# faustomorales/keras-ocr

Measured on AMD Instinct MI355X. Metric: images/sec end-to-end Pipeline.recognize() @768x768, higher is better.
Workload: dtype f32 (fp32 operands as 2 fp16 pieces [F(4,3) / head layers] or 3 bf16 pieces [1x1, dilated], 3 / 6 MFMA products, fp32 accumulate; fp32-class error vs fp64: tests/test_conv_gpu.py)

## Files before the change

### keras_ocr_amd/csrc/api.cpp

```cpp
#include "abi.h"
#include "taps.h"
#include <cmath>
#include <algorithm>
#include <mutex>
#include <set>

int arena_reserve(kocr_ctx* ctx, Arena& a, size_t bytes) {
  ctx->last_pl.valid = false;
  if (bytes <= a.cap) return KOCR_OK;
  if (a.base) {
    KOCR_HIP(ctx, hipStreamSynchronize(ctx->stream));
    KOCR_HIP(ctx, hipFree(a.base));
    a.base = nullptr;
    a.cap = 0;
  }
  const size_t want = bytes + (bytes >> 3) + 4096;
  void* p = nullptr;
  hipError_t e = hipMalloc(&p, want);
  if (e != hipSuccess) {
    ctx->set_err("workspace hipMalloc(" + std::to_string(want) + " B) failed: " + hipGetErrorString(e));
    return KOCR_ENOMEM;
  }
  a.base = (char*)p;
  a.cap = want;
// ... 88 lines not shown
  pending.push_back(pd);
  ProfRow& r = prof[name];
  r.launches += 1;
  r.flops += flops;
  r.bytes += bytes;
}

void kocr_ctx::prof_end() { hipEventRecord(pending.back().b, stream); }

int kocr_ctx::prof_flush() {
  if (pending.empty()) return KOCR_OK;
  KOCR_HIP(this, hipStreamSynchronize(stream));
  for (Pending& pd : pending) {
    float ms = 0.f;
    hipEventElapsedTime(&ms, pd.a, pd.b);
    prof[pd.name].ms += ms;
    ev_pool.push_back(pd.a);
    ev_pool.push_back(pd.b);
  }
  pending.clear();
  return KOCR_OK;
}

int craft_micro_batch(int micro_batch, int N, int H, int W) {
  int mb = micro_batch > 0 ? micro_batch : 32;
  while (mb > 1 && craft_workspace_bytes(mb, H, W) > ((size_t)96 << 30)) mb = (mb + 1) / 2;
  return std::min(mb, N);
}

long prepare_box_warps(kocr_ctx* ctx, const char* fn, int N, const float* boxes, const int32_t* counts, const void* out, int th,
                       int tw, std::vector<WarpParam>& prm) {
  const std::string f(fn);
  long M = 0;
  for (int i = 0; i < N; ++i) {
    if (counts[i] < 0) KOCR_FAIL(ctx, KOCR_EINVAL, f + ": negative count");
    M += counts[i];
  }
  if (M == 0) return 0;
  if (!boxes || !out) KOCR_FAIL(ctx, KOCR_EINVAL, f + ": null buffer");
  prm.resize((size_t)M);
  long m = 0;
  for (int i = 0; i < N; ++i)
    for (int j = 0; j < counts[i]; ++j, ++m) {
      const int rc = warp_prepare(boxes + m * 8, th, tw, &prm[m], nullptr);
      if (rc == 1) KOCR_FAIL(ctx, KOCR_EZERODIV, f + ": box with zero width or height (ZeroDivisionError at tools.py:95)");
      if (rc != 0) KOCR_FAIL(ctx, KOCR_EINVAL, f + ": singular perspective transform");
      prm[m].img = i;
    }
  return M;
}

extern "C" {

int kocr_create(kocr_ctx** out, int hip_device) {
  if (!out) return KOCR_EINVAL;
  *out = nullptr;
  int count = 0;
  if (hipGetDeviceCount(&count) != hipSuccess || hip_device < 0 || hip_device >= count) return KOCR_EHIP;
  if (hipSetDevice(hip_device) != hipSuccess) return KOCR_EHIP;
  kocr_ctx* c = new kocr_ctx();
  if (const char* e = getenv("KOCR_SPLIT"))
    c->split_mode = (!strcmp(e, "f16") || !strcmp(e, "fp16") || !strcmp(e, "f16x2")) ? KOCR_SPLIT_F16X2
                    : (!strcmp(e, "f16x1") || !strcmp(e, "fast"))                     ? KOCR_SPLIT_F16X1
                                                                                      : KOCR_SPLIT_BF16X3;
  {
    auto on = [](const char* name, bool dflt) {
      const char* e = getenv(name);
      return e ? atoi(e) != 0 : dflt;
    };
    c->sw.dense_splitk = on("KOCR_DENSE_SPLITK", true);
    c->sw.lstm16 = on("KOCR_LSTM16", true);
    c->sw.hs16 = on("KOCR_HS16", true);
    c->sw.k5 = on("KOCR_K5", true);
    c->sw.up2x = on("KOCR_UP2X", true);
    c->sw.w43h = on("KOCR_W43H", true);
    c->sw.w43 = on("KOCR_W43", true);
    c->sw.w43r = on("KOCR_W43R", true);
    c->sw.w43v = on("KOCR_W43V", true);
    c->sw.w43rag = on("KOCR_W43RAG", true);
    c->sw.w43dilh = on("KOCR_W43DILH", true);
    c->sw.cells = on("KOCR_CELLS", true);
    c->sw.wsplit = on("KOCR_WSPLIT", true);
    c->sw.dsplit = on("KOCR_DSPLIT", true);
    c->sw.hsplit = on("KOCR_HSPLIT", true);
    c->sw.first = on("KOCR_FIRST", true);
  }
  c->prof_layers = getenv("KOCR_PROF_LAYERS") != nullptr;
  if (const char* e = getenv("KOCR_LINFOLD")) c->opt_linfold = atoi(e) != 0;
  if (const char* e = getenv("KOCR_UPFOLD")) c->opt_upfold = atoi(e) != 0;
  c->device = hip_device;
  if (hipDeviceGetAttribute(&c->n_cu, hipDeviceAttributeMultiprocessorCount, hip_device) != hipSuccess ||
      hipStreamCreateWithFlags(&c->own_stream, hipStreamNonBlocking) != hipSuccess) {
    delete c;
    return KOCR_EHIP;
  }
  c->stream = c->own_stream;
  *out = c;
  return KOCR_OK;
}

void kocr_destroy(kocr_ctx* ctx) {
  if (!ctx) return;
  hipSetDevice(ctx->device);
  hipStreamSynchronize(ctx->stream);
  craft_free(ctx);
  crnn_free(ctx);
  for (void* p : ctx->owned) hipFree(p);
  for (Arena* a : {&ctx->ws, &ctx->pp, &ctx->pp2, &ctx->io, &ctx->pl, &ctx->bx})
    if (a->base) hipFree(a->base);
  for (auto& pd : ctx->pending) {
    hipEventDestroy(pd.a);
    hipEventDestroy(pd.b);
  }
  for (hipEvent_t e : ctx->ev_pool) hipEventDestroy(e);
  hipStreamDestroy(ctx->own_stream);
  delete ctx;
}

const char* kocr_last_error(const kocr_ctx* ctx) { return ctx ? ctx->err.c_str() : "null ctx"; }

int kocr_set_stream(kocr_ctx* ctx, void* hip_stream) {
  if (!ctx) return KOCR_EINVAL;
  KOCR_HIP(ctx, hipStreamSynchronize(ctx->stream));
  ctx->stream = hip_stream ? (hipStream_t)hip_stream : ctx->own_stream;
  return KOCR_OK;
}

int kocr_synchronize(kocr_ctx* ctx) {
  if (!ctx) return KOCR_EINVAL;
  KOCR_HIP(ctx, hipStreamSynchronize(ctx->stream));
  return KOCR_OK;
}

int kocr_device_alloc(kocr_ctx* ctx, void** out, uint64_t bytes) {
  if (!ctx || !out) return KOCR_EINVAL;
  KOCR_HIP(ctx, hipSetDevice(ctx->device));
  KOCR_HIP(ctx, hipMalloc(out, bytes ? bytes : 4));
  return KOCR_OK;
}

int kocr_device_free(kocr_ctx* ctx, void* p) {
  if (!ctx) return KOCR_EINVAL;
  KOCR_HIP(ctx, hipStreamSynchronize(ctx->stream));
  KOCR_HIP(ctx, hipFree(p));
  return KOCR_OK;
}

int kocr_memcpy_h2d(kocr_ctx* ctx, void* dst, const void* src, uint64_t bytes) {
  if (!ctx) return KOCR_EINVAL;
  KOCR_HIP(ctx, hipMemcpyAsync(dst, src, bytes, hipMemcpyHostToDevice, ctx->stream));
  KOCR_HIP(ctx, hipStreamSynchronize(ctx->stream));
  return KOCR_OK;
}

int kocr_memcpy_d2h(kocr_ctx* ctx, void* dst, const void* src, uint64_t bytes) {
  if (!ctx) return KOCR_EINVAL;
  KOCR_HIP(ctx, hipMemcpyAsync(dst, src, bytes, hipMemcpyDeviceToHost, ctx->stream));
  KOCR_HIP(ctx, hipStreamSynchronize(ctx->stream));
  return KOCR_OK;
}

int kocr_load_craft(kocr_ctx* ctx, int n, const char* const* names, const float* const* data,
                    const int64_t* shapes, const int* ranks) {
  if (!ctx || n <= 0 || !names || !data || !shapes || !ranks) return KOCR_EINVAL;
  KOCR_HIP(ctx, hipSetDevice(ctx->device));
  return craft_load(ctx, n, names, data, shapes, ranks);
// ... 617 lines not shown
```

### keras_ocr_amd/csrc/common.h

```cpp
#pragma once
#include <hip/hip_runtime.h>
#include <stdint.h>
#include <string>
#include <vector>
#include <map>
#include <atomic>
#include <cstdio>
#include <cstring>
#include "../../include/kocr.h"

#define KOCR_HIP(ctx, expr)                                                         \
  do {                                                                              \
    hipError_t _e = (expr);                                                         \
    if (_e != hipSuccess) {                                                         \
      (ctx)->set_err(std::string(#expr) + ": " + hipGetErrorString(_e) + " at " +   \
                     __FILE__ + ":" + std::to_string(__LINE__));                    \
      return KOCR_EHIP;                                                             \
    }                                                                               \
  } while (0)

#define KOCR_TRY(expr)            \
  do {                            \
    int _rc = (expr);             \
    if (_rc != KOCR_OK) return _rc; \
  } while (0)

#define KOCR_FAIL(ctx, code, msg) \
  do {                            \
    (ctx)->set_err(msg);          \
    return (code);                \
  } while (0)

struct Tensor {
  float* p = nullptr;
  int N = 0, H = 0, W = 0, C = 0;
  int cs = 0;
  int co = 0;
  unsigned* amax = nullptr;
  int Wv = 0;
  int wv() const { return Wv ? Wv : W; }
  int cellW = 0, cellWv = 0;
  int cells() const { return cellW ? W / cellW : 0; }
  size_t pixels() const { return (size_t)N * H * W; }
  Tensor slice(int off, int c) const {
    Tensor t = *this;
    t.co = co + off;
    t.C = c;
    return t;
  }
};

struct ConvLayer {
  std::string name;
  int Cin = 0, Cout = 0, KH = 1, KW = 1, dil = 1;
  int Kreal = 0, Kpad = 0, Cout_pad = 0, BN = 0;
  float* d_w = nullptr;
  float* d_pre_a = nullptr;
  float* d_pre_b = nullptr;
  float* d_post_a = nullptr;
  float* d_post_b = nullptr;
  int relu = 0;
  float* d_w_rgb4 = nullptr;
  unsigned short* d_ws = nullptr;
  int ws_cout_pad = 0;
  unsigned short* d_w4 = nullptr;
  int w4_cout_pad = 0;
  unsigned short* d_w4h = nullptr;
  float* d_pre_a_h = nullptr;
  unsigned short* d_ds = nullptr;
  int ds_cout_pad = 0;
  unsigned short* d_first = nullptr;
  float first_bound = 0.f;
  unsigned short* d_hs = nullptr;
  unsigned short* d_hs16 = nullptr;
  unsigned short* d_hsh = nullptr;
  std::vector<int> hs_wexp;
  unsigned short* d_k5 = nullptr;
  bool tap_inner = false;
  bool ready() const { return d_w != nullptr; }
};

struct ProfRow {
  int64_t launches = 0;
  double ms = 0, flops = 0, bytes = 0;
};

struct RangeRow {
  double launches = 0, elements = 0, nonzero = 0, below_m4 = 0, below_m14 = 0, sum_abs = 0, sum_abs_below_m4 = 0;
};

struct Arena {
  char* base = nullptr;
  size_t cap = 0, off = 0;
};

struct CraftNet;
struct CrnnNet;
struct Taps;

struct kocr_ctx {
  int device = 0;
  hipStream_t own_stream = nullptr;
  hipStream_t stream = nullptr;
  std::string err;
  void set_err(const std::string& s) { err = s; }

  int split_mode = KOCR_SPLIT_F16X2;
  bool opt_linfold = true, opt_upfold = true;
  int min_area_rect = KOCR_RECT_EXACT;
  struct Switches {
    bool dense_splitk = true;
    bool lstm16 = true;
    bool hs16 = true;
    bool k5 = true;
    bool up2x = true;
    bool w43h = true;
    bool w43 = true;
    bool w43r = true;
    bool w43v = true;
    bool w43rag = true;
    bool w43dilh = true;
    bool cells = true;
    bool wsplit = true;
    bool dsplit = true;
    bool hsplit = true;
    bool first = true;
  } sw;
  bool prof_layers = false;
  int n_cu = 0;

  unsigned* d_amax = nullptr;
  int amax_used = 0;
  static constexpr int AMAX_SLOTS = 1 << 16;
  int amax_begin();
  unsigned* amax_slots(int n);

  Arena ws, pp, pp2, io, pl;
  Arena bx;
  int ws_reserve(size_t bytes);
  void ws_reset() { ws.off = 0; }
  void* ws_alloc(size_t bytes);

  std::vector<void*> owned;
  int dev_alloc(void** out, size_t bytes);
  int upload(float** out, const std::vector<float>& host);
  void release(void* p);

  CraftNet* craft = nullptr;
  CrnnNet* crnn = nullptr;
  Taps* taps = nullptr;
  std::vector<std::string>* tap_rows = nullptr;

  struct LastPipeline {
    const float* d_boxes = nullptr;
    const int32_t* d_counts = nullptr;
    const int32_t* d_labels = nullptr;
    int N = 0, cap = 0, M = 0;
    bool valid = false;
  } last_pl;

  bool range_on = false;
  void* d_range = nullptr;
  std::map<std::string, RangeRow> range;

  bool prof_on = false;
  std::map<std::string, ProfRow> prof;
  struct Pending {
    std::string name;
    hipEvent_t a, b;
  };
  std::vector<Pending> pending;
  std::vector<hipEvent_t> ev_pool;
  hipEvent_t get_event();
  void prof_begin(const char* name, double flops, double bytes);
  void prof_end();
  int prof_flush();
};

int arena_reserve(kocr_ctx* ctx, Arena& a, size_t bytes);
inline void* arena_alloc(Arena& a, size_t bytes) {
  const size_t o = (a.off + 255) & ~(size_t)255;
  if (o + bytes > a.cap) return nullptr;
  a.off = o + bytes;
  return a.base + o;
}
inline void* kocr_ctx::ws_alloc(size_t bytes) { return arena_alloc(ws, bytes); }

struct ProfScope {
  kocr_ctx* c;
  ProfScope(kocr_ctx* ctx, const char* name, double flops, double bytes) : c(ctx) {
    if (c->tap_rows) c->tap_rows->push_back(name);
    if (c->prof_on) c->prof_begin(name, flops, bytes);
  }
  ~ProfScope() {
    if (c->prof_on) c->prof_end();
  }
};

inline std::string prof_name(const kocr_ctx* ctx, const ConvLayer& L, const std::string& row, const std::string& layer_row) {
  return ctx->prof_layers ? layer_row + ":" + L.name : row;
}

template <auto K, typename P>
int launch_persistent(kocr_ctx* ctx, const P& p, int total_tiles, int block, int lds, int attr_lds, int occ = 1,
                      int* grid_out = nullptr) {
  static std::atomic<bool> attr_done[64];
  const int dev = ctx->device & 63;
// ... 162 lines not shown
```

### keras_ocr_amd/csrc/conv_dsplit.hip

```cpp
#include "split_common.h"
#include "w43_common.h"
#include "probe_clock.h"
#include <cmath>
#include <algorithm>

struct DsParams {
  const float* in;
  const unsigned short* wgt;
  float* out;
  const float* pre_a;
  const float* pre_b;
  const float* post_a;
  const float* post_b;
  int H, W, Cin, in_cs, in_co;
  int Cout, Cout_pad, out_cs, out_co;
  int relu;
  int KH, KW, dil;
  int nsteps;
  int Mtotal;
  int total_tiles;
  const unsigned* amax_in;
  int w_exp;
  unsigned* amax_out;
  const float* up;
  int up_H, up_W;
  float up_sy, up_sx;
  unsigned dv_hw[2];
};


template <int WM, int WN, int HALF, int UP, int PAIR = 0>
__global__ __launch_bounds__(128 * WM * WN, WM * WN == 2 ? 2 : 1) void conv_ds_kernel(DsParams p) {
  constexpr int NP = HALF ? 2 : 3;
  constexpr int NCW = WM * WN;
  constexpr int NMT = 8 * WM;
  constexpr int TILE_PX = 256 * WM;
  constexpr int PXI = 16 * NCW;
  constexpr int IPT = TILE_PX / PXI;
  constexpr int KH_STRIDE = 256;
  constexpr int PLANE = NMT * 2 * KH_STRIDE;
  constexpr int BUF = NP * PLANE;
  extern __shared__ __attribute__((aligned(16))) unsigned short As[];
  const int tid = threadIdx.x, lane = tid & 63;
  const int wave = __builtin_amdgcn_readfirstlane(tid >> 6);
  const int l31 = lane & 31, l5 = lane >> 5;
  const int nblk_n = p.Cout_pad / (32 * WN);
  const int total = p.total_tiles;
  const int ns = p.nsteps;
  const int G = gridDim.x;
  const int pad_y = p.dil * (p.KH / 2), pad_x = p.dil * (p.KW / 2);

  if (wave >= NCW) {
    const int ptid = tid - 64 * NCW;
    const int quad = ptid & 3;
    constexpr unsigned OOB = 0x80000000u;
    const float in_scale = HALF ? kocr_pow2(kocr_scale_exp(p.amax_in, 13)) : 1.f;
    (void)in_scale;
    int ldst[IPT];
#pragma unroll
    for (int it = 0; it < IPT; ++it) {
      const int idx = (ptid >> 2) + it * PXI;
      ldst[it] = ((idx >> 5) * 2 + (quad >> 1)) * KH_STRIDE + ((((idx & 31) * 8) ^ ((quad >> 1) * 32)) + (quad & 1) * 4);
    }
    int L_ld = blockIdx.x, ld_ky = 0, ld_kx = 0, ld_cg = 0;
    unsigned goff[IPT];
    int gy[IPT], gx[IPT];
    bool gok[IPT];
    __amdgpu_buffer_rsrc_t rsrc;
    auto tile_geometry = [&]() __attribute__((always_inline)) {
      const int tile = kocr_xcd_remap(L_ld < total ? L_ld : 0, total);
      const long pm0 = (long)(tile / nblk_n) * TILE_PX;
      const float* bbase_v = p.in + (pm0 * p.in_cs + p.in_co) - (long)(pad_y * p.W + pad_x) * p.in_cs;
      const unsigned long long bb = (unsigned long long)bbase_v;
      const unsigned long long bbu = ((unsigned long long)(unsigned)__builtin_amdgcn_readfirstlane((int)(bb >> 32)) << 32) |
                                     (unsigned)__builtin_amdgcn_readfirstlane((int)bb);
      rsrc = __builtin_amdgcn_make_buffer_rsrc((void*)bbu, 0, 0x80000000, 0x00020000);
#pragma unroll
      for (int it = 0; it < IPT; ++it) {
        const int idx = (ptid >> 2) + it * PXI;
        const long g = pm0 + idx;
        gok[it] = g < p.Mtotal && L_ld < total;
        gx[it] = (int)(g % p.W);
        gy[it] = (int)((g / p.W) % p.H);
        goff[it] = (unsigned)((idx * p.in_cs + quad * 4) * 4);
      }
    };
    auto load_raw2 = [&](v4f (&ra)[IPT], v4f (&rb)[IPT]) __attribute__((always_inline)) {
      const int soff = ld_cg * 64;
#pragma unroll
      for (int it = 0; it < IPT; ++it) {
        const unsigned off = gok[it] ? goff[it] : OOB;
        ra[it] = __builtin_bit_cast(v4f, __builtin_amdgcn_raw_buffer_load_b128(rsrc, off, soff, 0));
        rb[it] = __builtin_bit_cast(v4f, __builtin_amdgcn_raw_buffer_load_b128(rsrc, off, soff + 64, 0));
      }
      ld_cg += 2;
      if (ld_cg == p.Cin / 16) {
        ld_cg = 0;
        L_ld += G;
        tile_geometry();
      }
    };
    auto load_raw = [&](v4f (&raw)[IPT]) __attribute__((always_inline)) {
      const int dy = ld_ky * p.dil - pad_y, dx = ld_kx * p.dil - pad_x;
      const int soff = (((dy + pad_y) * p.W + (dx + pad_x)) * p.in_cs + ld_cg * 16) * 4;
#pragma unroll
      for (int it = 0; it < IPT; ++it) {
        const bool ok = gok[it] && (unsigned)(gy[it] + dy) < (unsigned)p.H && (unsigned)(gx[it] + dx) < (unsigned)p.W;
        raw[it] = __builtin_bit_cast(v4f, __builtin_amdgcn_raw_buffer_load_b128(rsrc, ok ? goff[it] : OOB, soff, 0));
      }
      if (++ld_kx == p.KW) {
        ld_kx = 0;
        if (++ld_ky == p.KH) {
          ld_ky = 0;
          if (++ld_cg == p.Cin / 16) {
            ld_cg = 0;
            L_ld += G;
            tile_geometry();
          }
        }
      }
    };
    auto produce = [&](const v4f (&raw)[IPT], int buf) __attribute__((always_inline)) {
      unsigned short* base = As + buf * BUF;
#pragma unroll
      for (int it = 0; it < IPT; ++it) {
        unsigned short* dst = base + ldst[it];
        if constexpr (HALF) {
          u2v h, l;
          kocr_split4_h(raw[it] * in_scale, h, l);
          *reinterpret_cast<u2v*>(dst) = h;
          *reinterpret_cast<u2v*>(dst + PLANE) = l;
        } else {
          u2v h, m, l;
          kocr_split4(raw[it], h, m, l);
          *reinterpret_cast<u2v*>(dst) = h;
          *reinterpret_cast<u2v*>(dst + PLANE) = m;
          *reinterpret_cast<u2v*>(dst + 2 * PLANE) = l;
        }
      }
    };
    const int my_tiles = (total - (int)blockIdx.x + G - 1) / G;
    const int T = my_tiles * ns;
    tile_geometry();
    constexpr int D = PAIR ? 6 : 4;
    v4f raw[D][IPT];
    int k = 0;
    if constexpr (PAIR) {
      load_raw2(raw[0], raw[1]);
      load_raw2(raw[2], raw[3]);
      PROBE_T0();
      for (; k + D <= T; k += D) {
#pragma unroll
        for (int d = 0; d < D; d += 2) {
          load_raw2(raw[(d + 4) % D], raw[(d + 5) % D]);
          PROBE_T(6);
          produce(raw[d], 0);
          PROBE_T(4);
          __syncthreads();
          PROBE_T(5);
          produce(raw[d + 1], 1);
          PROBE_T(4);
          __syncthreads();
          PROBE_T(5);
        }
      }
      PROBE_TEND(tid == 64 * NCW, 4, 7);
#pragma unroll
      for (int d = 0; d < 4; ++d)
        if (k + d < T) {
          produce(raw[d], d & 1);
          __syncthreads();
        }
    } else {
#pragma unroll
    for (int d = 0; d < D - 1; ++d) load_raw(raw[d]);
    PROBE_T0();
    for (; k + D <= T; k += D) {
#pragma unroll
      for (int d = 0; d < D; ++d) {
        load_raw(raw[(d + D - 1) % D]);
        PROBE_T(6);
        produce(raw[d], d & 1);
        PROBE_T(4);
        __syncthreads();
        PROBE_T(5);
      }
    }
    PROBE_TEND(tid == 64 * NCW, 4, 7);
#pragma unroll
    for (int d = 0; d < D - 1; ++d)
      if (k + d < T) {
        produce(raw[d], d & 1);
        __syncthreads();
      }
    }
    __syncthreads();
    return;
  }

  const int wn = (WN == 4) ? wave : (wave % WN), wm = (WM == 1) ? 0 : (wave / WN);
  const int ntiles32 = p.Cout_pad >> 5;
  const size_t w_step = (size_t)ntiles32 * NP * 64 * 8;
  auto w_tile = [&](int nt) { return p.wgt + ((size_t)(nt * WN + wn) * NP * 64 + lane) * 8; };

  bf8 bw[NP], bwn[NP];
  f16v acc[4][2];
  const int a_lane = (wm * 8 * 2 + l5) * KH_STRIDE + ((l31 * 8) ^ (l5 * 32));
  auto load_a = [&](bf8 (&a)[2][NP], const unsigned short* bufp, int g) __attribute__((always_inline)) {
    const unsigned short* base = bufp + a_lane + g * 4 * KH_STRIDE;
#pragma unroll
    for (int m = 0; m < 2; ++m)
#pragma unroll
      for (int s = 0; s < NP; ++s) a[m][s] = *reinterpret_cast<const bf8*>(base + s * PLANE + m * 2 * KH_STRIDE);
  };
  auto mfma6 = [&](const bf8 (&a)[2][NP], int g) __attribute__((always_inline)) {
    if constexpr (HALF) {
      const hf8 b0 = __builtin_bit_cast(hf8, bw[0]), b1 = __builtin_bit_cast(hf8, bw[1]);
#pragma unroll
      for (int m = 0; m < 2; ++m)
        acc[g][m] = __builtin_amdgcn_mfma_f32_32x32x16_f16(__builtin_bit_cast(hf8, a[m][1]), b0, acc[g][m], 0, 0, 0);
// ... 3 lines not shown
#pragma unroll
      for (int m = 0; m < 2; ++m)
        acc[g][m] = __builtin_amdgcn_mfma_f32_32x32x16_f16(__builtin_bit_cast(hf8, a[m][0]), b0, acc[g][m], 0, 0, 0);
    } else {
      const bf8 b0 = bw[0], b1 = bw[1], b2 = bw[NP - 1];
#pragma unroll
      for (int m = 0; m < 2; ++m) acc[g][m] = __builtin_amdgcn_mfma_f32_32x32x16_bf16(a[m][NP - 1], b0, acc[g][m], 0, 0, 0);
#pragma unroll
      for (int m = 0; m < 2; ++m) acc[g][m] = __builtin_amdgcn_mfma_f32_32x32x16_bf16(a[m][0], b2, acc[g][m], 0, 0, 0);
#pragma unroll
      for (int m = 0; m < 2; ++m) acc[g][m] = __builtin_amdgcn_mfma_f32_32x32x16_bf16(a[m][1], b1, acc[g][m], 0, 0, 0);
#pragma unroll
      for (int m = 0; m < 2; ++m) acc[g][m] = __builtin_amdgcn_mfma_f32_32x32x16_bf16(a[m][1], b0, acc[g][m], 0, 0, 0);
#pragma unroll
      for (int m = 0; m < 2; ++m) acc[g][m] = __builtin_amdgcn_mfma_f32_32x32x16_bf16(a[m][0], b1, acc[g][m], 0, 0, 0);
#pragma unroll
      for (int m = 0; m < 2; ++m) acc[g][m] = __builtin_amdgcn_mfma_f32_32x32x16_bf16(a[m][0], b0, acc[g][m], 0, 0, 0);
    }
  };
  bf8 a0[2][NP], a1[2][NP];
  auto compute_step = [&](auto last_c, const unsigned short* bufp, const unsigned short* bufn,
                          const unsigned short* w_next) __attribute__((always_inline)) {
    constexpr bool LAST = decltype(last_c)::value;
#pragma unroll
    for (int s = 0; s < NP; ++s) bwn[s] = *reinterpret_cast<const bf8*>(w_next + (size_t)s * 64 * 8);
    load_a(a1, bufp, 1);
    __builtin_amdgcn_sched_barrier(0);
    mfma6(a0, 0);
    __builtin_amdgcn_sched_barrier(0);
    load_a(a0, bufp, 2);
    __builtin_amdgcn_sched_barrier(0);
    mfma6(a1, 1);
    __builtin_amdgcn_sched_barrier(0);
    load_a(a1, bufp, 3);
    __builtin_amdgcn_sched_barrier(0);
    mfma6(a0, 2);
    __builtin_amdgcn_sched_barrier(0);
    __syncthreads();
    if constexpr (!LAST) load_a(a0, bufn, 0);
    __builtin_amdgcn_sched_barrier(0);
    mfma6(a1, 3);
    __builtin_amdgcn_sched_barrier(0);
#pragma unroll
    for (int s = 0; s < NP; ++s) bw[s] = bwn[s];
  };

  int gs = 0;
  {
    const int tile0 = kocr_xcd_remap(blockIdx.x, total);
    const unsigned short* w0 = w_tile(tile0 % nblk_n);
#pragma unroll
    for (int s = 0; s < NP; ++s) bw[s] = *reinterpret_cast<const bf8*>(w0 + (size_t)s * 64 * 8);
  }
  __syncthreads();
  load_a(a0, As, 0);
  PROBE_T0();
  for (int L = blockIdx.x; L < total; L += G) {
    const int tile = kocr_xcd_remap(L, total);
    const int mt = tile / nblk_n, nt = tile - mt * nblk_n;
    const long pm0 = (long)mt * TILE_PX;
    const unsigned short* w_ptr = w_tile(nt);
    const unsigned short* w_after = (L + G < total) ? w_tile(kocr_xcd_remap(L + G, total) % nblk_n) : w_ptr;
#pragma unroll
    for (int g = 0; g < 4; ++g)
#pragma unroll
      for (int m = 0; m < 2; ++m)
#pragma unroll
        for (int r = 0; r < 16; ++r) acc[g][m][r] = 0.f;
    __builtin_amdgcn_s_waitcnt(0x0F70);
    if constexpr (UP != 0) {
      for (int s = 0; s < ns - 1; ++s, ++gs)
        compute_step(std::false_type{}, As + (gs & 1) * BUF, As + ((gs + 1) & 1) * BUF, w_ptr + (size_t)(s + 1) * w_step);
      compute_step(std::true_type{}, As + (gs & 1) * BUF, As + ((gs + 1) & 1) * BUF, w_after);
      ++gs;
    } else {
      for (int s = 0; s < ns; ++s, ++gs)
        compute_step(std::false_type{}, As + (gs & 1) * BUF, As + ((gs + 1) & 1) * BUF, s + 1 < ns ? w_ptr + (size_t)(s + 1) * w_step : w_after);
    }
    PROBE_T(0);

    {
      const int n = (nt * WN + wn) * 32 + l31;
      const int nc = n < p.Cout ? n : p.Cout - 1;
      const float unscale = HALF ? kocr_pow2(-(kocr_scale_exp(p.amax_in, 13) + p.w_exp)) : 1.f;
      const float pa = p.pre_a[nc] * unscale, pb = p.pre_b[nc];
      const bool has_post = p.post_a != nullptr;
      const float qa = has_post ? p.post_a[nc] : 1.f, qb = has_post ? p.post_b[nc] : 0.f;
      if constexpr (UP) {
        unsigned* tab = reinterpret_cast<unsigned*>(As + 2 * BUF) + wave * (256 * 8);
        const long wbase = pm0 + (long)wm * 256;
        const unsigned ucs4 = (unsigned)p.Cout * 4u;
        const int hw = p.H * p.W;
        const long wb = wbase < (long)p.Mtotal - 1 ? wbase : (long)p.Mtotal - 1;
        const int n0 = __builtin_amdgcn_readfirstlane((int)(wb / hw));
#pragma unroll
        for (int i = 0; i < 4; ++i) {
          const int q = lane + 64 * i;
          long gl = wbase + q;
          if (gl > (long)p.Mtotal - 1) gl = (long)p.Mtotal - 1;
          const int gi = (int)gl;
          const int ox = gi % p.W, t2 = gi / p.W;
          const int oy = t2 % p.H, ni = t2 / p.H;
          const float fy = ((float)oy + 0.5f) * p.up_sy - 0.5f;
          const float fx = ((float)ox + 0.5f) * p.up_sx - 0.5f;
          const float fly = floorf(fy), flx = floorf(fx);
          const int y0 = max((int)fly, 0), y1 = min((int)ceilf(fy), p.up_H - 1);
          const int x0 = max((int)flx, 0), x1 = min((int)ceilf(fx), p.up_W - 1);
          const unsigned r0 = (unsigned)(((ni - n0) * p.up_H + y0) * p.up_W), r1 = (unsigned)(((ni - n0) * p.up_H + y1) * p.up_W);
          uint4 o4;
          o4.x = (r0 + x0) * ucs4;
          o4.y = (r0 + x1) * ucs4;
          o4.z = (r1 + x0) * ucs4;
          o4.w = (r1 + x1) * ucs4;
          *reinterpret_cast<uint4*>(tab + q * 8) = o4;
          float2 wl;
          wl.x = fx - flx;
          wl.y = fy - fly;
          *reinterpret_cast<float2*>(tab + q * 8 + 4) = wl;
        }
        __builtin_amdgcn_fence(__ATOMIC_SEQ_CST, "wavefront");
        __builtin_amdgcn_wave_barrier();
        const unsigned long long ub = (unsigned long long)(p.up + (size_t)n0 * p.up_H * p.up_W * p.Cout);
        const unsigned long long ubu = ((unsigned long long)(unsigned)__builtin_amdgcn_readfirstlane((int)(ub >> 32)) << 32) |
                                       (unsigned)__builtin_amdgcn_readfirstlane((int)ub);
        const __amdgpu_buffer_rsrc_t ru = __builtin_amdgcn_make_buffer_rsrc((void*)ubu, 0, 0x7FFFFFFF, 0x00020000);
        const unsigned ch = (unsigned)nc * 4u;
        if constexpr (UP == 2) {
          float tb[2][4][8];
          unsigned tab_lane = 4 * l5 * 8;
          asm volatile("" : "+v"(tab_lane));
          const unsigned* tab_l = tab + tab_lane;
          auto up_issue = [&](int gm, float (&v)[4][8]) __attribute__((always_inline)) {
#pragma unroll
            for (int rr = 0; rr < 4; ++rr) {
              const unsigned* e = tab_l + (gm * 32 + 8 * rr) * 8;
              const uint4 oa = *reinterpret_cast<const uint4*>(e);
              const uint4 od = *reinterpret_cast<const uint4*>(e + 3 * 8);
              v[rr][0] = __uint_as_float(__builtin_amdgcn_raw_buffer_load_b32(ru, oa.x + ch, 0, 0));
              v[rr][1] = __uint_as_float(__builtin_amdgcn_raw_buffer_load_b32(ru, oa.y + ch, 0, 0));
              v[rr][2] = __uint_as_float(__builtin_amdgcn_raw_buffer_load_b32(ru, od.x + ch, 0, 0));
              v[rr][3] = __uint_as_float(__builtin_amdgcn_raw_buffer_load_b32(ru, od.y + ch, 0, 0));
              v[rr][4] = __uint_as_float(__builtin_amdgcn_raw_buffer_load_b32(ru, oa.z + ch, 0, 0));
              v[rr][5] = __uint_as_float(__builtin_amdgcn_raw_buffer_load_b32(ru, oa.w + ch, 0, 0));
              v[rr][6] = __uint_as_float(__builtin_amdgcn_raw_buffer_load_b32(ru, od.z + ch, 0, 0));
              v[rr][7] = __uint_as_float(__builtin_amdgcn_raw_buffer_load_b32(ru, od.w + ch, 0, 0));
            }
          };
          auto up_blend = [&](f16v& a, int gm, const float (&v)[4][8]) __attribute__((always_inline)) {
#pragma unroll
            for (int rr = 0; rr < 4; ++rr) {
              const unsigned* e = tab_l + (gm * 32 + 8 * rr) * 8;
#pragma unroll
              for (int j = 0; j < 4; ++j) {
                const float2 wl = *reinterpret_cast<const float2*>(e + j * 8 + 4);
                const int c0 = (j + 1) >> 1;
                const float top = v[rr][c0] + (v[rr][c0 + 1] - v[rr][c0]) * wl.x;
                const float bot = v[rr][4 + c0] + (v[rr][4 + c0 + 1] - v[rr][4 + c0]) * wl.x;
                a[rr * 4 + j] += top + (bot - top) * wl.y;
              }
            }
          };
          up_issue(0, tb[0]);
#pragma unroll
          for (int gm = 0; gm < 8; ++gm) {
            if (gm + 1 < 8) up_issue(gm + 1, tb[(gm + 1) & 1]);
            __builtin_amdgcn_sched_barrier(0);
            up_blend(acc[gm >> 1][gm & 1], gm, tb[gm & 1]);
            __builtin_amdgcn_sched_barrier(0);
          }
        } else {
// ... 50 lines not shown
        const unsigned w0 = (unsigned)(pm0 + (long)wm * 256);
        const unsigned wend = w0 + 256 < (unsigned)p.Mtotal ? w0 + 256 : (unsigned)p.Mtotal;
        if (wend > w0) {
          const unsigned hw = (unsigned)(p.H * p.W);
          const int n_lo = __builtin_amdgcn_readfirstlane((int)w4_fdiv(w0, p.dv_hw)),
                    n_hi = __builtin_amdgcn_readfirstlane((int)w4_fdiv(wend - 1, p.dv_hw));
          if (n_lo == n_hi && wend == w0 + 256) {
            float mx = 0.f;
#pragma unroll
            for (int g = 0; g < 4; ++g)
#pragma unroll
              for (int m = 0; m < 2; ++m)
#pragma unroll
                for (int r = 0; r < 16; ++r) mx = fmaxf(mx, fabsf(acc[g][m][r]));
            kocr_amax_update(p.amax_out + n_lo, n < p.Cout ? mx : 0.f);
          } else {
            int l5o = 4 * l5;
            asm volatile("" : "+v"(l5o));
            for (int ni = n_lo; ni <= n_hi; ++ni) {
              const unsigned i0 = (unsigned)ni * hw, i1 = i0 + hw;
              const int lo_r = (int)((i0 > w0 ? i0 : w0) - w0), hi_r = (int)((i1 < wend ? i1 : wend) - w0);
              float mx = 0.f;
#pragma unroll
              for (int g = 0; g < 4; ++g)
#pragma unroll
                for (int m = 0; m < 2; ++m)
#pragma unroll
                  for (int r = 0; r < 16; ++r) {
                    const int rel = (g * 2 + m) * 32 + (r & 3) + 8 * (r >> 2) + l5o;
                    if (rel >= lo_r && rel < hi_r) mx = fmaxf(mx, fabsf(acc[g][m][r]));
                  }
              kocr_amax_update(p.amax_out + ni, n < p.Cout ? mx : 0.f);
            }
          }
        }
      }
      PROBE_T(2);
      const int ocs4 = p.out_cs * 4;
      const long rem = ((long)p.Mtotal - pm0) * ocs4;
      const unsigned long long bb = (unsigned long long)(p.out + (pm0 * p.out_cs + p.out_co));
      const unsigned long long bbu = ((unsigned long long)(unsigned)__builtin_amdgcn_readfirstlane((int)(bb >> 32)) << 32) |
                                     (unsigned)__builtin_amdgcn_readfirstlane((int)bb);
      const __amdgpu_buffer_rsrc_t ro = __builtin_amdgcn_make_buffer_rsrc(
          (void*)bbu, 0, __builtin_amdgcn_readfirstlane((int)(rem < 0x7FFFFFFFL ? rem : 0x7FFFFFFFL)), 0x00020000);
      const unsigned vo = n < p.Cout ? (unsigned)((4 * l5 * p.out_cs + n) * 4) : 0x80000000u;
#pragma unroll
      for (int g = 0; g < 4; ++g)
#pragma unroll
        for (int m = 0; m < 2; ++m)
#pragma unroll
          for (int r = 0; r < 16; ++r) {
            const int px = ((wm * 4 + g) * 2 + m) * 32 + (r & 3) + 8 * (r >> 2);
            __builtin_amdgcn_raw_buffer_store_b32(__float_as_uint(acc[g][m][r]), ro, vo, px * ocs4, 0);
          }
      PROBE_T(3);
    }
    if constexpr (UP != 0) load_a(a0, As + (gs & 1) * BUF, 0);
  }
  PROBE_TEND(tid == 0, 0, 4);
}

int prepare_dsplit(kocr_ctx* ctx, ConvLayer& L, const float* w, bool w_is_oihw) {
  if (L.Cin % 16 != 0 || L.Cout <= 32 || (L.KH == 3 && L.KW == 3 && L.dil == 1)) return KOCR_OK;
  const int Cin = L.Cin, Cout = L.Cout, ntaps = L.KH * L.KW;
  const int wcls = Cout > 64 ? 128 : 64;
  const int cp = (Cout + wcls - 1) / wcls * wcls;
  const int nt32 = cp / 32;
  std::vector<unsigned short> u((size_t)(Cin / 16) * ntaps * nt32 * 3 * 64 * 8, 0);
  for (int c = 0; c < Cin; ++c)
    for (int tap = 0; tap < ntaps; ++tap)
      for (int o = 0; o < Cout; ++o) {
        const float g = w_is_oihw ? w[((size_t)o * Cin + c) * ntaps + tap] : w[((size_t)tap * Cin + c) * Cout + o];
        const int k = c % 16, lane = (k >> 3) * 32 + (o & 31), j = k & 7;
        const size_t step = (size_t)(c / 16) * ntaps + tap;
        unsigned short pc[3];
        kocr_split3_host(g, pc);
        for (int s = 0; s < 3; ++s) u[(((step * nt32 + o / 32) * 3 + s) * 64 + lane) * 8 + j] = pc[s];
      }
  L.ds_cout_pad = cp;
  void* d = nullptr;
  KOCR_TRY(ctx->dev_alloc(&d, u.size() * sizeof(unsigned short)));
  KOCR_HIP(ctx, hipMemcpy(d, u.data(), u.size() * sizeof(unsigned short), hipMemcpyHostToDevice));
  L.d_ds = (unsigned short*)d;

  return KOCR_OK;
}

bool dsplit_usable(const kocr_ctx* ctx, const ConvLayer& L, const Tensor& in) {
  return ctx->sw.dsplit && L.d_ds && in.cs % 4 == 0 && in.co % 4 == 0 && ((uintptr_t)in.p & 15) == 0 &&
         (size_t)in.pixels() * in.cs < ((size_t)1 << 40);
}

bool dsplit_applicable(const kocr_ctx* ctx, const ConvLayer& L, const Tensor& in) {
  return dsplit_usable(ctx, L, in) && in.pixels() >= 4096;
}

template <int WM, int WN, int HALF, int UP = 0, int PAIR = 0>
static int ds_launch(kocr_ctx* ctx, DsParams& p, size_t M) {
  constexpr int NCW = WM * WN;
  constexpr int LDS_BYTES = 2 * (HALF ? 2 : 3) * (8 * WM) * 2 * 256 * 2 + (UP ? NCW * 256 * 32 : 0);
  const size_t mtiles = (M + 256 * WM - 1) / (256 * WM);
  p.total_tiles = (int)(mtiles * (p.Cout_pad / (32 * WN)));
  int grid;
  PROBE_RESET(ctx);
  KOCR_TRY((launch_persistent<conv_ds_kernel<WM, WN, HALF, UP, PAIR>>(ctx, p, p.total_tiles, 128 * NCW, LDS_BYTES, LDS_BYTES,
                                                                       NCW == 2 ? 2 : 1, &grid)));
  {
    char what[64];
    snprintf(what, sizeof what, "conv_ds<%d,%d,%d,pair%d> tiles %d steps %d", WM, WN, UP, PAIR, p.total_tiles, p.nsteps);
    (void)what;
    PROBE_REPORT(ctx, what, grid);
  }
  return KOCR_OK;
}

int launch_conv_dsplit(kocr_ctx* ctx, const ConvLayer& L, const Tensor& in, const Tensor& out, const Tensor* up) {
  const size_t M = in.pixels();
  DsParams p;
  p.in = in.p;
  p.wgt = L.d_ds;
  p.out = out.p;
  p.pre_a = L.d_pre_a;
  p.pre_b = L.d_pre_b;
  p.post_a = L.d_post_a;
  p.post_b = L.d_post_b;
  p.H = in.H;
  p.W = in.W;
  p.Cin = L.Cin;
  p.in_cs = in.cs;
  p.in_co = in.co;
  p.Cout = L.Cout;
  p.Cout_pad = L.ds_cout_pad;
  p.out_cs = out.cs;
  p.out_co = out.co;
  p.relu = L.relu;
  p.KH = L.KH;
  p.KW = L.KW;
  p.dil = L.dil;
  p.nsteps = L.KH * L.KW * (L.Cin / 16);
  p.Mtotal = (int)M;
  p.total_tiles = 0;
  p.amax_out = out.amax;
  const bool half = false;
  p.up = nullptr;
  p.up_H = p.up_W = 0;
  p.up_sy = p.up_sx = 0.f;
  if (up) {
    if (half || up->C != L.Cout || up->cs != L.Cout || up->co != 0 || up->N != in.N || L.KH != 1 || L.KW != 1 ||
        2 * (size_t)up->H * up->W * L.Cout * 4 >= ((size_t)1 << 31))
      KOCR_FAIL(ctx, KOCR_EINVAL, "conv " + L.name + ": unsupported up-sampled addend");
    p.up = up->p;
    p.up_H = up->H;
    p.up_W = up->W;
    p.up_sy = (float)up->H / (float)in.H;
    p.up_sx = (float)up->W / (float)in.W;
  }
  p.amax_in = nullptr;
  p.w_exp = 0;
  w4_div_magic((unsigned)(in.H * in.W), p.dv_hw);
  const int wcls = L.Cout > 64 ? 128 : 64;
  const std::string row = std::string("conv_d") + (half ? "h" : "s") + "_" + std::to_string(wcls == 128 ? 256 : 512) + "x" +
                          std::to_string(wcls) + (up ? "_up" : "");
  const std::string nm = prof_name(ctx, L, row, row);
  const double flops = 2.0 * (double)M * L.Kreal * L.Cout;
  const double bytes = 4.0 * ((double)M * L.Cin + (double)M * L.Cout + (double)L.Kreal * L.Cout + (up ? (double)up->pixels() * L.Cout : 0.0));
  ProfScope ps(ctx, nm.c_str(), flops, bytes);
  const bool line_pairs = L.KH == 1 && L.KW == 1 && (L.Cin / 16) % 2 == 0 && in.cs % 32 == 0 && in.co % 32 == 0;
  if (up) {
    const bool no_up2 = !ctx->sw.up2x;
    if (!no_up2 && in.H == 2 * up->H && in.W == 2 * up->W && in.W % 4 == 0) {
      if (line_pairs) return wcls == 128 ? ds_launch<1, 4, 0, 2, 1>(ctx, p, M) : ds_launch<2, 2, 0, 2, 1>(ctx, p, M);
      return wcls == 128 ? ds_launch<1, 4, 0, 2>(ctx, p, M) : ds_launch<2, 2, 0, 2>(ctx, p, M);
    }
    return wcls == 128 ? ds_launch<1, 4, 0, 1>(ctx, p, M) : ds_launch<2, 2, 0, 1>(ctx, p, M);
  }
  if (line_pairs) return wcls == 128 ? ds_launch<1, 4, 0, 0, 1>(ctx, p, M) : ds_launch<2, 2, 0, 0, 1>(ctx, p, M);
  return wcls == 128 ? ds_launch<1, 4, 0>(ctx, p, M) : ds_launch<2, 2, 0>(ctx, p, M);
}
```

### keras_ocr_amd/csrc/conv_mfma.hip

```cpp
#include "common.h"
#include <cmath>
#include <type_traits>

typedef float f32x16 __attribute__((ext_vector_type(16)));
typedef float v4f __attribute__((ext_vector_type(4)));

struct ConvParams {
  const float* in;
  const uint8_t* in_u8;
  const float* lut;
  const float* wgt;
  float* out;
  const float* pre_a;
  const float* pre_b;
  const float* post_a;
  const float* post_b;
  int H, W, Cin, in_cs, in_co;
  int Cout, Cout_pad, out_cs, out_co;
  int KH, KW, dil, padh, padw;
  int relu;
  int Mtotal;
  int Kreal, nchunks;
  float* pool_out;
  int pool_cs, pool_co, write_full, tiles_per_row;
// ... 299 lines not shown
    const float qa = has_post ? p.post_a[nc] : 1.f;
    const float qb = has_post ? p.post_b[nc] : 0.f;
#pragma unroll
    for (int i = 0; i < TM; ++i) {
      if constexpr (POOL) {
#pragma unroll
        for (int g = 0; g < 4; ++g) {
          const int ml = wm * WTM + i * 32 + 8 * g + 4 * lk;
          float best = -INFINITY;
#pragma unroll
          for (int e = 0; e < 4; ++e) {
            float v = acc[i][j][4 * g + e] * pa + pb;
            if (p.relu) v = fmaxf(v, 0.f);
            if (has_post) v = v * qa + qb;
            best = fmaxf(best, v);
            if (p.write_full && live) {
              const long pix = pm0 + (long)(e >> 1) * p.W + 2 * (ml >> 2) + (e & 1);
              p.out[pix * p.out_cs + p.out_co + n] = v;
            }
          }
          const long nimg = pm0 / ((long)p.H * p.W);
          const long pp = (nimg * (p.H >> 1) + (y0t >> 1)) * (p.W >> 1) + (x0t >> 1) + (ml >> 2);
          if (live) p.pool_out[pp * p.pool_cs + p.pool_co + n] = best;
        }
      } else {
#pragma unroll
        for (int r = 0; r < 16; ++r) {
          float v = acc[i][j][r] * pa + pb;
          if (p.relu) v = fmaxf(v, 0.f);
          if (has_post) v = v * qa + qb;
          acc[i][j][r] = v;
        }
      }
    }
    if (p.amax_out || p.amax_pool) {
      float mx = 0.f;
      if constexpr (!POOL) {
#pragma unroll
        for (int i = 0; i < TM; ++i)
#pragma unroll
          for (int r = 0; r < 16; ++r) mx = fmaxf(mx, fabsf(acc[i][j][r]));
      } else {
#pragma unroll
        for (int i = 0; i < TM; ++i)
#pragma unroll
          for (int r = 0; r < 16; ++r) {
            float v = acc[i][j][r] * pa + pb;
            if (p.relu) v = fmaxf(v, 0.f);
            if (has_post) v = v * qa + qb;
            mx = fmaxf(mx, fabsf(v));
          }
      }
      mx = live ? mx : 0.f;
      if (p.amax_out) kocr_amax_update(p.amax_out, mx);
      if (p.amax_pool) kocr_amax_update(p.amax_pool, mx);
    }
    if constexpr (!POOL) {
      const int ocs4 = p.out_cs * 4;
      const long rem = ((long)p.Mtotal - m0) * ocs4;
      const unsigned long long bb = (unsigned long long)(p.out + ((long)m0 * p.out_cs + p.out_co));
      const unsigned long long bbu = ((unsigned long long)(unsigned)__builtin_amdgcn_readfirstlane((int)(bb >> 32)) << 32) |
                                     (unsigned)__builtin_amdgcn_readfirstlane((int)bb);
      const __amdgpu_buffer_rsrc_t ro = __builtin_amdgcn_make_buffer_rsrc(
          (void*)bbu, 0, __builtin_amdgcn_readfirstlane((int)(rem < 0x7FFFFFFFL ? rem : 0x7FFFFFFFL)), 0x00020000);
      const unsigned vo = live ? (unsigned)((4 * lk * p.out_cs + n) * 4) : 0x80000000u;
#pragma unroll
      for (int i = 0; i < TM; ++i)
#pragma unroll
        for (int r = 0; r < 16; ++r) {
          const int px = wm * WTM + i * 32 + (r & 3) + 8 * (r >> 2);
          __builtin_amdgcn_raw_buffer_store_b32(__float_as_uint(acc[i][j][r]), ro, vo, px * ocs4, 0);
        }
    }
  }
}

static int round_up(int a, int b) { return (a + b - 1) / b * b; }

int prepare_conv(kocr_ctx* ctx, ConvLayer& L, const float* w, bool w_is_oihw, int Cin, int Cout,
                 int KH, int KW, int dil, const float* pre_a, const float* pre_b, int relu,
                 const float* post_a, const float* post_b) {
  {
    void* old[] = {L.d_w, L.d_pre_a, L.d_pre_b, L.d_post_a, L.d_post_b, L.d_w_rgb4, L.d_pre_a_h, L.d_ws, L.d_w4,
                   L.d_w4h, L.d_ds, L.d_first, L.d_hs, L.d_hs16, L.d_hsh, L.d_k5};
    bool any = false;
    for (void* q : old) any = any || q != nullptr;
    if (any) {
      KOCR_HIP(ctx, hipStreamSynchronize(ctx->stream));
      for (void* q : old) ctx->release(q);
    }
  }
  L.d_w = L.d_pre_a = L.d_pre_b = L.d_post_a = L.d_post_b = L.d_w_rgb4 = L.d_pre_a_h = nullptr;
  L.d_ws = L.d_w4 = L.d_w4h = L.d_ds = L.d_first = L.d_hs = L.d_hs16 = L.d_hsh = L.d_k5 = nullptr;
  L.hs_wexp.clear();
  L.first_bound = 0.f;
  L.Cin = Cin;
  L.Cout = Cout;
  L.KH = KH;
  L.KW = KW;
  L.dil = dil;
  L.relu = relu;
  L.Kreal = KH * KW * Cin;
  L.tap_inner = (Cin % 16 == 0);
  L.Kpad = round_up(L.Kreal, 32);
  L.BN = Cout > 64 ? 128 : (Cout > 32 ? 64 : 32);
  L.Cout_pad = round_up(Cout, L.BN);
  std::vector<float> wp((size_t)L.Kpad * L.Cout_pad, 0.f);
  for (int ky = 0; ky < KH; ++ky)
    for (int kx = 0; kx < KW; ++kx)
      for (int c = 0; c < Cin; ++c)
        for (int o = 0; o < Cout; ++o) {
          const float v = w_is_oihw ? w[(((size_t)o * Cin + c) * KH + ky) * KW + kx]
                                    : w[(((size_t)ky * KW + kx) * Cin + c) * Cout + o];
          const int tap = ky * KW + kx;
          const size_t row = L.tap_inner ? (size_t)((c / 16) * KH * KW + tap) * 16 + (c % 16) : (size_t)tap * Cin + c;
          wp[row * L.Cout_pad + o] = v;
        }
  KOCR_TRY(ctx->upload(&L.d_w, wp));
  KOCR_TRY(prepare_wsplit(ctx, L, w, w_is_oihw));
  KOCR_TRY(prepare_w43(ctx, L, w, w_is_oihw));
  KOCR_TRY(prepare_w43h(ctx, L, w, w_is_oihw, pre_a));
  KOCR_TRY(prepare_dsplit(ctx, L, w, w_is_oihw));
  KOCR_TRY(prepare_hsplit(ctx, L, w, w_is_oihw));
  KOCR_TRY(prepare_k5(ctx, L, w, w_is_oihw));
  KOCR_TRY(prepare_first(ctx, L, w, w_is_oihw));
  if (Cin == 3 && KH == 3 && KW == 3 && dil == 1) {
    std::vector<float> w4((size_t)48 * L.Cout_pad, 0.f);
    for (int tap = 0; tap < 9; ++tap)
      for (int c = 0; c < 3; ++c)
        for (int o = 0; o < Cout; ++o)
          w4[(size_t)(tap * 4 + c) * L.Cout_pad + o] =
              w_is_oihw ? w[(((size_t)o * 3 + c) * 3 + tap / 3) * 3 + tap % 3] : w[((size_t)tap * 3 + c) * Cout + o];
    KOCR_TRY(ctx->upload(&L.d_w_rgb4, w4));
  }
  std::vector<float> a(L.Cout_pad, 1.f), b(L.Cout_pad, 0.f);
  for (int o = 0; o < Cout; ++o) {
    if (pre_a) a[o] = pre_a[o];
    if (pre_b) b[o] = pre_b[o];
  }
  KOCR_TRY(ctx->upload(&L.d_pre_a, a));
  KOCR_TRY(ctx->upload(&L.d_pre_b, b));
  if (L.d_first) {
    const double xmax[3] = {0.515 / 0.229, 0.544 / 0.224, 0.594 / 0.225};
    double bound = 0;
    for (int o = 0; o < Cout; ++o) {
      double sw = 0;
      for (int ky = 0; ky < KH; ++ky)
        for (int kx = 0; kx < KW; ++kx)
          for (int c = 0; c < Cin; ++c)
            sw += std::fabs((double)(w_is_oihw ? w[(((size_t)o * Cin + c) * KH + ky) * KW + kx] : w[(((size_t)ky * KW + kx) * Cin + c) * Cout + o])) * xmax[c % 3];
      double v = std::fabs((double)a[o]) * sw + std::fabs((double)b[o]);
      if (post_a || post_b) v = std::fabs(post_a ? (double)post_a[o] : 1.0) * v + std::fabs(post_b ? (double)post_b[o] : 0.0);
      bound = std::max(bound, v);
    }
    L.first_bound = (float)(bound * (1.0 + 1e-6));
  }
  if (L.d_hsh && !L.d_pre_a_h) {
    std::vector<float> ah(L.Cout_pad, 1.f);
    for (int o = 0; o < Cout; ++o) ah[o] = std::ldexp(a[o], -L.hs_wexp[o]);
    KOCR_TRY(ctx->upload(&L.d_pre_a_h, ah));
  }
  L.d_post_a = L.d_post_b = nullptr;
  if (post_a || post_b) {
    std::vector<float> qa(L.Cout_pad, 1.f), qb(L.Cout_pad, 0.f);
    for (int o = 0; o < Cout; ++o) {
      if (post_a) qa[o] = post_a[o];
      if (post_b) qb[o] = post_b[o];
    }
    KOCR_TRY(ctx->upload(&L.d_post_a, qa));
    KOCR_TRY(ctx->upload(&L.d_post_b, qb));
  }
  return KOCR_OK;
}

template <int BM, int BN, int WM, int WN, int BK, int PF>
static void dispatch_mode(int mode, dim3 grid, hipStream_t s, const ConvParams& p) {
// ... 142 lines not shown
```

Baseline: 262.2.

## Enable fp16x2 split path for 1x1 upsample-add dsplit convs with per-image scaling

Adds a half-precision (two fp16 pieces) variant of the dsplit 1x1 conv kernel for wide-output layers with an upsampled addend. The old path used three bf16 pieces. Per-image activation scale exponents are kept in an LDS table, and per-output-channel weight exponents are prepacked on the host, so the split is taken per image and later undone in the epilogue. This cuts MFMA products from 6 to 3 and shrinks LDS traffic, at the cost of extra epilogue scaling, per-tile index divisions, and a range-dependent accuracy risk.

```diff
diff --git a/keras_ocr_amd/csrc/api.cpp b/keras_ocr_amd/csrc/api.cpp
--- a/keras_ocr_amd/csrc/api.cpp
+++ b/keras_ocr_amd/csrc/api.cpp
@@ -194,6 +194,7 @@
     c->sw.cells = on("KOCR_CELLS", true);
     c->sw.wsplit = on("KOCR_WSPLIT", true);
     c->sw.dsplit = on("KOCR_DSPLIT", true);
+    c->sw.dsh = on("KOCR_DSH", true);
     c->sw.hsplit = on("KOCR_HSPLIT", true);
     c->sw.first = on("KOCR_FIRST", true);
   }
diff --git a/keras_ocr_amd/csrc/common.h b/keras_ocr_amd/csrc/common.h
--- a/keras_ocr_amd/csrc/common.h
+++ b/keras_ocr_amd/csrc/common.h
@@ -69,6 +69,8 @@
   float* d_pre_a_h = nullptr;
   unsigned short* d_ds = nullptr;
   int ds_cout_pad = 0;
+  unsigned short* d_dsh = nullptr;
+  float* d_ds_wsc = nullptr;
   unsigned short* d_first = nullptr;
   float first_bound = 0.f;
   unsigned short* d_hs = nullptr;
@@ -123,6 +125,7 @@
     bool cells = true;
     bool wsplit = true;
     bool dsplit = true;
+    bool dsh = true;
     bool hsplit = true;
     bool first = true;
   } sw;
diff --git a/keras_ocr_amd/csrc/conv_dsplit.hip b/keras_ocr_amd/csrc/conv_dsplit.hip
--- a/keras_ocr_amd/csrc/conv_dsplit.hip
+++ b/keras_ocr_amd/csrc/conv_dsplit.hip
@@ -20,13 +20,16 @@
   int Mtotal;
   int total_tiles;
   const unsigned* amax_in;
-  int w_exp;
+  const float* wsc;
+  int nimg;
   unsigned* amax_out;
   const float* up;
   int up_H, up_W;
   float up_sy, up_sx;
   unsigned dv_hw[2];
 };
+
+constexpr int DS_MAX_IMG = 64;
 
 
 template <int WM, int WN, int HALF, int UP, int PAIR = 0>
@@ -49,13 +52,16 @@
   const int ns = p.nsteps;
   const int G = gridDim.x;
   const int pad_y = p.dil * (p.KH / 2), pad_x = p.dil * (p.KW / 2);
+  int* e_tab = reinterpret_cast<int*>(As + 2 * BUF) + (UP ? NCW * 256 * 8 : 0);
+  if constexpr (HALF) {
+    for (int i = tid; i < p.nimg; i += 128 * NCW) e_tab[i] = kocr_scale_exp(p.amax_in + i, 13);
+    __syncthreads();
+  }
 
   if (wave >= NCW) {
     const int ptid = tid - 64 * NCW;
     const int quad = ptid & 3;
     constexpr unsigned OOB = 0x80000000u;
-    const float in_scale = HALF ? kocr_pow2(kocr_scale_exp(p.amax_in, 13)) : 1.f;
-    (void)in_scale;
     int ldst[IPT];
 #pragma unroll
     for (int it = 0; it < IPT; ++it) {
@@ -120,6 +126,19 @@
         }
       }
     };
+    float isc[IPT];
+    int L_pr = blockIdx.x, s_pr = 0;
+    auto scale_geometry = [&]() __attribute__((always_inline)) {
+      const int tile = kocr_xcd_remap(L_pr < total ? L_pr : 0, total);
+      const unsigned pm0 = (unsigned)(tile / nblk_n) * TILE_PX;
+#pragma unroll
+      for (int it = 0; it < IPT; ++it) {
+        const unsigned g = pm0 + (unsigned)((ptid >> 2) + it * PXI);
+        const int ni = (int)w4_fdiv(g < (unsigned)p.Mtotal ? g : (unsigned)p.Mtotal - 1, p.dv_hw);
+        isc[it] = kocr_pow2(e_tab[ni]);
+      }
+    };
+    if constexpr (HALF) scale_geometry();
     auto produce = [&](const v4f (&raw)[IPT], int buf) __attribute__((always_inline)) {
       unsigned short* base = As + buf * BUF;
 #pragma unroll
@@ -127,7 +146,7 @@
         unsigned short* dst = base + ldst[it];
         if constexpr (HALF) {
           u2v h, l;
-          kocr_split4_h(raw[it] * in_scale, h, l);
+          kocr_split4_h(raw[it] * isc[it], h, l);
           *reinterpret_cast<u2v*>(dst) = h;
           *reinterpret_cast<u2v*>(dst + PLANE) = l;
         } else {
@@ -136,6 +155,13 @@
           *reinterpret_cast<u2v*>(dst) = h;
           *reinterpret_cast<u2v*>(dst + PLANE) = m;
           *reinterpret_cast<u2v*>(dst + 2 * PLANE) = l;
+        }
+      }
+      if constexpr (HALF) {
+        if (++s_pr == ns) {
+          s_pr = 0;
+          L_pr += G;
+          scale_geometry();
         }
       }
     };
@@ -305,10 +331,49 @@
     {
       const int n = (nt * WN + wn) * 32 + l31;
       const int nc = n < p.Cout ? n : p.Cout - 1;
-      const float unscale = HALF ? kocr_pow2(-(kocr_scale_exp(p.amax_in, 13) + p.w_exp)) : 1.f;
-      const float pa = p.pre_a[nc] * unscale, pb = p.pre_b[nc];
+      const float pa = p.pre_a[nc], pb = p.pre_b[nc];
       const bool has_post = p.post_a != nullptr;
       const float qa = has_post ? p.post_a[nc] : 1.f, qb = has_post ? p.post_b[nc] : 0.f;
+      if constexpr (HALF) {
+        const unsigned w0 = (unsigned)(pm0 + (long)wm * 256);
+        const unsigned wl = w0 + 255 < (unsigned)p.Mtotal ? w0 + 255 : (unsigned)p.Mtotal - 1;
+        const int n_lo = __builtin_amdgcn_readfirstlane((int)w4_fdiv(w0 < (unsigned)p.Mtotal ? w0 : wl, p.dv_hw)),
+                  n_hi = __builtin_amdgcn_readfirstlane((int)w4_fdiv(wl, p.dv_hw));
+        if (n_lo == n_hi) {
+          const float fi = kocr_pow2(-e_tab[n_lo]);
+#pragma unroll
+          for (int g = 0; g < 4; ++g)
+#pragma unroll
+            for (int m = 0; m < 2; ++m)
+#pragma unroll
+              for (int r = 0; r < 16; ++r) acc[g][m][r] *= fi;
+        } else {
+          const unsigned hw = (unsigned)(p.H * p.W);
+          int l5o = 4 * l5;
+          asm volatile("" : "+v"(l5o));
+          for (int ni = n_lo; ni <= n_hi; ++ni) {
+            const unsigned i0 = (unsigned)ni * hw, i1 = i0 + hw;
+            const int lo_r = (int)((i0 > w0 ? i0 : w0) - w0), hi_r = (int)(i1 - w0);
+            const float fi = kocr_pow2(-e_tab[ni]);
+#pragma unroll
+            for (int g = 0; g < 4; ++g)
+#pragma unroll
+              for (int m = 0; m < 2; ++m)
+#pragma unroll
+                for (int r = 0; r < 16; ++r) {
+                  const int rel = (g * 2 + m) * 32 + (r & 3) + 8 * (r >> 2) + l5o;
+                  if (rel >= lo_r && rel < hi_r) acc[g][m][r] *= fi;
+                }
+          }
+        }
+        const float fo = p.wsc[n];
+#pragma unroll
+        for (int g = 0; g < 4; ++g)
+#pragma unroll
+          for (int m = 0; m < 2; ++m)
+#pragma unroll
+            for (int r = 0; r < 16; ++r) acc[g][m][r] *= fo;
+      }
       if constexpr (UP) {
         unsigned* tab = reinterpret_cast<unsigned*>(As + 2 * BUF) + wave * (256 * 8);
         const long wbase = pm0 + (long)wm * 256;
@@ -525,7 +590,38 @@
   KOCR_TRY(ctx->dev_alloc(&d, u.size() * sizeof(unsigned short)));
   KOCR_HIP(ctx, hipMemcpy(d, u.data(), u.size() * sizeof(unsigned short), hipMemcpyHostToDevice));
   L.d_ds = (unsigned short*)d;
-
+  if (ntaps == 1 && Cout > 64) {
+    std::vector<float> wsc(cp, 1.f);
+    std::vector<int> wexp(Cout, 0);
+    for (int o = 0; o < Cout; ++o) {
+      float wmax = 0.f;
+      for (int c = 0; c < Cin; ++c) wmax = std::max(wmax, std::fabs(w_is_oihw ? w[(size_t)o * Cin + c] : w[(size_t)c * Cout + o]));
+      if (wmax > 0.f && std::isfinite(wmax)) {
+        int E;
+        std::frexp(wmax, &E);
+        wexp[o] = std::max(-100, std::min(100, 15 - E));
+      }
+      wsc[o] = std::ldexp(1.f, -wexp[o]);
+    }
+    std::vector<unsigned short> v((size_t)(Cin / 16) * nt32 * 2 * 64 * 8, 0);
+    for (int c = 0; c < Cin; ++c)
+      for (int o = 0; o < Cout; ++o) {
+        const float g = std::ldexp(w_is_oihw ? w[(size_t)o * Cin + c] : w[(size_t)c * Cout + o], wexp[o]);
+        const int k = c % 16, lane = (k >> 3) * 32 + (o & 31), j = k & 7;
+        const size_t step = c / 16;
+        const _Float16 h = (_Float16)g, l = (_Float16)(g - (float)h);
+        unsigned short hb, lb;
+        memcpy(&hb, &h, 2);
+        memcpy(&lb, &l, 2);
+        v[(((step * nt32 + o / 32) * 2 + 0) * 64 + lane) * 8 + j] = hb;
+        v[(((step * nt32 + o / 32) * 2 + 1) * 64 + lane) * 8 + j] = lb;
+      }
+    void* dh = nullptr;
+    KOCR_TRY(ctx->dev_alloc(&dh, v.size() * sizeof(unsigned short)));
+    KOCR_HIP(ctx, hipMemcpy(dh, v.data(), v.size() * sizeof(unsigned short), hipMemcpyHostToDevice));
+    L.d_dsh = (unsigned short*)dh;
+    KOCR_TRY(ctx->upload(&L.d_ds_wsc, wsc));
+  }
   return KOCR_OK;
 }
 
@@ -541,7 +637,7 @@
 template <int WM, int WN, int HALF, int UP = 0, int PAIR = 0>
 static int ds_launch(kocr_ctx* ctx, DsParams& p, size_t M) {
   constexpr int NCW = WM * WN;
-  constexpr int LDS_BYTES = 2 * (HALF ? 2 : 3) * (8 * WM) * 2 * 256 * 2 + (UP ? NCW * 256 * 32 : 0);
+  constexpr int LDS_BYTES = 2 * (HALF ? 2 : 3) * (8 * WM) * 2 * 256 * 2 + (UP ? NCW * 256 * 32 : 0) + (HALF ? DS_MAX_IMG * 4 : 0);
   const size_t mtiles = (M + 256 * WM - 1) / (256 * WM);
   p.total_tiles = (int)(mtiles * (p.Cout_pad / (32 * WN)));
   int grid;
@@ -550,7 +646,7 @@
                                                                        NCW == 2 ? 2 : 1, &grid)));
   {
     char what[64];
-    snprintf(what, sizeof what, "conv_ds<%d,%d,%d,pair%d> tiles %d steps %d", WM, WN, UP, PAIR, p.total_tiles, p.nsteps);
+    snprintf(what, sizeof what, "conv_ds<%d,%d,%d,%d,pair%d> tiles %d steps %d", WM, WN, HALF, UP, PAIR, p.total_tiles, p.nsteps);
     (void)what;
     PROBE_REPORT(ctx, what, grid);
   }
@@ -584,12 +680,14 @@
   p.Mtotal = (int)M;
   p.total_tiles = 0;
   p.amax_out = out.amax;
-  const bool half = false;
+  const int wcls = L.Cout > 64 ? 128 : 64;
+  const bool half = up && wcls == 128 && ctx->split_mode != KOCR_SPLIT_BF16X3 && ctx->sw.dsh && L.d_dsh && L.d_ds_wsc &&
+                    in.amax && in.N >= 1 && in.N <= DS_MAX_IMG && L.KH == 1 && L.KW == 1;
   p.up = nullptr;
   p.up_H = p.up_W = 0;
   p.up_sy = p.up_sx = 0.f;
   if (up) {
-    if (half || up->C != L.Cout || up->cs != L.Cout || up->co != 0 || up->N != in.N || L.KH != 1 || L.KW != 1 ||
+    if (up->C != L.Cout || up->cs != L.Cout || up->co != 0 || up->N != in.N || L.KH != 1 || L.KW != 1 ||
         2 * (size_t)up->H * up->W * L.Cout * 4 >= ((size_t)1 << 31))
       KOCR_FAIL(ctx, KOCR_EINVAL, "conv " + L.name + ": unsupported up-sampled addend");
     p.up = up->p;
@@ -599,9 +697,15 @@
     p.up_sx = (float)up->W / (float)in.W;
   }
   p.amax_in = nullptr;
-  p.w_exp = 0;
+  p.wsc = nullptr;
+  p.nimg = in.N;
+  if (half) {
+    p.wgt = L.d_dsh;
+    p.wsc = L.d_ds_wsc;
+    p.amax_in = in.amax;
+    if (ctx->range_on) KOCR_TRY(launch_range_stats(ctx, L.name, in, in.amax, 13));
+  }
   w4_div_magic((unsigned)(in.H * in.W), p.dv_hw);
-  const int wcls = L.Cout > 64 ? 128 : 64;
   const std::string row = std::string("conv_d") + (half ? "h" : "s") + "_" + std::to_string(wcls == 128 ? 256 : 512) + "x" +
                           std::to_string(wcls) + (up ? "_up" : "");
   const std::string nm = prof_name(ctx, L, row, row);
@@ -611,7 +715,12 @@
   const bool line_pairs = L.KH == 1 && L.KW == 1 && (L.Cin / 16) % 2 == 0 && in.cs % 32 == 0 && in.co % 32 == 0;
   if (up) {
     const bool no_up2 = !ctx->sw.up2x;
-    if (!no_up2 && in.H == 2 * up->H && in.W == 2 * up->W && in.W % 4 == 0) {
+    const bool up2 = !no_up2 && in.H == 2 * up->H && in.W == 2 * up->W && in.W % 4 == 0;
+    if (half) {
+      if (up2) return line_pairs ? ds_launch<1, 4, 1, 2, 1>(ctx, p, M) : ds_launch<1, 4, 1, 2>(ctx, p, M);
+      return ds_launch<1, 4, 1, 1>(ctx, p, M);
+    }
+    if (up2) {
       if (line_pairs) return wcls == 128 ? ds_launch<1, 4, 0, 2, 1>(ctx, p, M) : ds_launch<2, 2, 0, 2, 1>(ctx, p, M);
       return wcls == 128 ? ds_launch<1, 4, 0, 2>(ctx, p, M) : ds_launch<2, 2, 0, 2>(ctx, p, M);
     }
diff --git a/keras_ocr_amd/csrc/conv_mfma.hip b/keras_ocr_amd/csrc/conv_mfma.hip
--- a/keras_ocr_amd/csrc/conv_mfma.hip
+++ b/keras_ocr_amd/csrc/conv_mfma.hip
@@ -405,7 +405,7 @@
                  const float* post_a, const float* post_b) {
   {
     void* old[] = {L.d_w, L.d_pre_a, L.d_pre_b, L.d_post_a, L.d_post_b, L.d_w_rgb4, L.d_pre_a_h, L.d_ws, L.d_w4,
-                   L.d_w4h, L.d_ds, L.d_first, L.d_hs, L.d_hs16, L.d_hsh, L.d_k5};
+                   L.d_w4h, L.d_ds, L.d_dsh, L.d_ds_wsc, L.d_first, L.d_hs, L.d_hs16, L.d_hsh, L.d_k5};
     bool any = false;
     for (void* q : old) any = any || q != nullptr;
     if (any) {
@@ -414,7 +414,8 @@
     }
   }
   L.d_w = L.d_pre_a = L.d_pre_b = L.d_post_a = L.d_post_b = L.d_w_rgb4 = L.d_pre_a_h = nullptr;
-  L.d_ws = L.d_w4 = L.d_w4h = L.d_ds = L.d_first = L.d_hs = L.d_hs16 = L.d_hsh = L.d_k5 = nullptr;
+  L.d_ws = L.d_w4 = L.d_w4h = L.d_ds = L.d_dsh = L.d_first = L.d_hs = L.d_hs16 = L.d_hsh = L.d_k5 = nullptr;
+  L.d_ds_wsc = nullptr;
   L.hs_wexp.clear();
   L.first_bound = 0.f;
   L.Cin = Cin;
```

Result: no change. 263.6 (median of 6 runs) (+0.6%).
